# BelledonneCommunications/mediastreamer2

Measured on AMD Instinct MI355X. Metric: concurrent 48 kHz streams/node at <10 ms tick; Mpix/s YUV scale, higher is better.
Workload: dtype f32

## Files before the change

### mediastreamer2_amd/csrc/aec_steps.hpp

```cpp

template <int F_>
struct Wave {
	static constexpr int F = F_, K = F / 64, G = 64, NBL = 1;
	using Seq = WSeq<K>;
	__device__ static __forceinline__ int lane() { return threadIdx.x; }
	__device__ static __forceinline__ float first(float v) { return rdlane(v, 0); }
	__device__ static __forceinline__ float last(float v) { return rdlane(v, 63); }
	__device__ static __forceinline__ float shr1(float head, float v) {
		float t = __shfl_up(v, 1);
		if (threadIdx.x == 0) t = head;
		return t;
	}
	__device__ static __forceinline__ int any(bool p) { return __any(p); }
	template <typename Op>
	__device__ static __forceinline__ float tree(float v, Op op) { return wave_tree(v, op); }
	__device__ static __forceinline__ void dc_notch(const float (&in)[K], float radius, float den2, float &m0, float &m1, float (&out)[K]) {
		w_dc_notch<K>(in, radius, den2, m0, m1, out);
	}
	__device__ static __forceinline__ void deemphasis(const float (&d)[K], float &mem, float (&out)[K]) { w_deemphasis<K>(d, mem, out); }
	template <typename LL, typename LT>
	__device__ static __forceinline__ void rfft_forward(LL &L, const LT &T, float2 (&out)[K], const float *src = nullptr) {
		w_rfft_forward<F>(L, T, out, src);
	}
	template <typename LL, typename LT>
	__device__ static __forceinline__ void rfft_inverse(LL &L, const LT &T, const float2 (&in)[K]) { w_rfft_inverse<F>(L, T, in); }
	__device__ static __forceinline__ float band_total(const float (&vb)[NBL], float *) {
		float sum = 0;
#pragma unroll
		for (int i = 0; i < NB_BANDS; ++i) sum = sum + rdlane(vb[0], i);
		return sum;
	}
};

template <typename P, typename LL, typename LT>
__device__ __forceinline__ void far_end(LL &L, const LT &T, const float (&far)[P::K], const float (&xp)[P::K], float &memX, float (&xn)[P::K],
                                        float2 (&X0)[P::K], float &Sxx) {
	constexpr int K = P::K, F = P::F;
	const int e0 = P::lane() * K;
	float prev = P::shr1(memX, far[K - 1]);
#pragma unroll
	for (int k = 0; k < K; ++k) {
		xn[k] = far[k] - .9f * prev;
		prev = far[k];
	}
	memX = P::last(far[K - 1]);
	Sxx = P::Seq::inner_prod(xn, xn);
	WSYNC();
	store_vec<K>(L.tbuf + e0, xp);
	store_vec<K>(L.tbuf + F + e0, xn);
	P::rfft_forward(L, T, X0);
}

template <typename P>
__device__ __forceinline__ auto near_end(const float (&fin)[P::K], float radius, AecScalars &sc, float (&input)[P::K]) {
	constexpr int K = P::K;
	bool satl = false;
#pragma unroll
	for (int k = 0; k < K; ++k) satl |= (fin[k] <= -32000.f || fin[k] >= 32000.f);
	const auto any_sat = P::any(satl);
	const float den2 = (float)(radius * radius + .7 * (1 - radius) * (1 - radius));
	float v[K];
	P::dc_notch(fin, radius, den2, sc.notch0, sc.notch1, v);
	float vprev = P::shr1(sc.memD, v[K - 1]);
#pragma unroll
	for (int k = 0; k < K; ++k) {
		input[k] = v[k] - .9f * vprev;
		vprev = v[k];
	}
	sc.memD = P::last(v[K - 1]);
	return any_sat;
}

template <typename P>
__device__ __forceinline__ void bin_power(const float2 (&X)[P::K], float (&pw)[P::K], float &pw_F) {
	constexpr int K = P::K;
	const int e0 = P::lane() * K;
	float nyq = 0;
#pragma unroll
	for (int k = 0; k < K; ++k) {
		if (e0 + k == 0) {
			pw[k] = X[k].x * X[k].x;
			nyq = X[k].y * X[k].y;
		} else {
			pw[k] = X[k].x * X[k].x + X[k].y * X[k].y;
		}
	}
	pw_F = P::first(nyq);
}

template <typename P, typename TW, typename TX>
__device__ __forceinline__ void gradient(TW (&w)[P::K], const TX (&x)[P::K], float prop, const float2 (&E)[P::K], const float (&pp)[P::K], float pp_F) {
	constexpr int K = P::K;
	const int e0 = P::lane() * K;
#pragma unroll
	for (int k = 0; k < K; ++k) {
		const v2f xv = {x[k].x, x[k].y}, ev = {E[k].x, E[k].y};
		const float Wt = prop * pp[k];
		v2f st = pk_cmul_conj(xv, ev) * (v2f){Wt, Wt};
		if (k == 0) {
			const v2f dc = (xv * ev) * (v2f){Wt, prop * pp_F};
			if (e0 == 0) st = dc;
		}
		const v2f r = (v2f){w[k].x, w[k].y} + st;
		w[k].x = r.x, w[k].y = r.y;
	}
}

template <typename P, typename LL, typename LT, typename TW>
__device__ __forceinline__ void constrain(LL &L, const LT &T, TW (&wv)[P::K]) {
	constexpr int K = P::K, F = P::F;
	const int e0 = P::lane() * K;
	float2 w[K];
#pragma unroll
	for (int k = 0; k < K; ++k) w[k] = make_float2(wv[k].x, wv[k].y);
	P::rfft_inverse(L, T, w);
	float z[K];
#pragma unroll
	for (int k = 0; k < K; ++k) z[k] = 0.f;
	store_vec<K>(w_time(L) + F + e0, z);
	P::rfft_forward(L, T, w, w_time(L));
#pragma unroll
	for (int k = 0; k < K; ++k) wv[k].x = w[k].x, wv[k].y = w[k].y;
}

__device__ __forceinline__ bool two_path_update(AecScalars &sc, float Sff, float See, float Dbf) {
	sc.Davg1 = .6f * sc.Davg1 + .4f * (Sff - See);
	sc.Davg2 = .85f * sc.Davg2 + .15f * (Sff - See);
	sc.Dvar1 = .36f * sc.Dvar1 + (.4f * Sff) * (.4f * Dbf);
	sc.Dvar2 = .7225f * sc.Dvar2 + (.15f * Sff) * (.15f * Dbf);
	bool update_foreground = false;
	if ((Sff - See) * fabsf(Sff - See) > Sff * Dbf) update_foreground = true;
	else if (sc.Davg1 * fabsf(sc.Davg1) > .5f * sc.Dvar1) update_foreground = true;
	else if (sc.Davg2 * fabsf(sc.Davg2) > .25f * sc.Dvar2) update_foreground = true;
	if (update_foreground) {
		sc.fg_updates++;
		sc.Davg1 = sc.Davg2 = 0;
		sc.Dvar1 = sc.Dvar2 = 0;
	}
	return update_foreground;
}
template <typename P>
__device__ __forceinline__ void blend_foreground(const float *hann, float (&efg)[P::K], const float (&ybg)[P::K]) {
	constexpr int K = P::K, F = P::F;
	const int e0 = P::lane() * K;
	float h0[K], h1[K];
	load_vec<K>(hann + e0, h0);
	load_vec<K>(hann + F + e0, h1);
#pragma unroll
	for (int k = 0; k < K; ++k) efg[k] = h1[k] * efg[k] + h0[k] * ybg[k];
}
__device__ __forceinline__ bool two_path_reset(AecScalars &sc, float Sff, float See, float Dbf) {
	bool reset_background = false;
	if ((-(Sff - See)) * fabsf(Sff - See) > 4.f * (Sff * Dbf)) reset_background = true;
	if ((-sc.Davg1) * fabsf(sc.Davg1) > 4.f * sc.Dvar1) reset_background = true;
	if ((-sc.Davg2) * fabsf(sc.Davg2) > 4.f * sc.Dvar2) reset_background = true;
	if (reset_background) {
		sc.bg_resets++;
		sc.Davg1 = sc.Davg2 = 0;
		sc.Dvar1 = sc.Dvar2 = 0;
	}
	return reset_background;
}
template <typename P>
__device__ __forceinline__ void take_foreground(const float (&efg)[P::K], const float (&input)[P::K], float Sff, float (&ybg)[P::K], float (&e2)[P::K],
                                                float &See) {
#pragma unroll
	for (int k = 0; k < P::K; ++k) {
		ybg[k] = efg[k];
		e2[k] = input[k] - efg[k];
	}
	See = Sff;
}

template <typename P, typename TS>
__device__ __forceinline__ void output_and_correlations(AecScalars &sc, const float (&input)[P::K], const float (&efg)[P::K], const float (&e2)[P::K],
                                                        const float (&ybg)[P::K], TS any_sat, int (&out_i)[P::K], float &Sey, float &Syy, float &Sdd) {
	constexpr int K = P::K;
	{
		float d[K], tout[K];
#pragma unroll
		for (int k = 0; k < K; ++k) d[k] = input[k] - efg[k];
		P::deemphasis(d, sc.memE, tout);
#pragma unroll
// ... 359 lines not shown
```

### mediastreamer2_amd/csrc/aec_tick.hpp

```cpp

struct SmallLayout {
	int XPREV;
	int E;
	int POWER;
	int POWER1, EH, YH;
	int LASTY;
	int ECHON, INBUF, OUTBUF, NOISE, OLDPS, ZETA, S_, SMIN, STMP;
	int MISC;
	int PROP;
	int WNORM;
	int TAIL;
	int OLDPS_B;
	int ZETA_B;
	int FGNORM;
	int TOTAL;
};
__host__ __device__ constexpr SmallLayout small_layout(int F) {
	SmallLayout l{};
	l.XPREV = 0, l.E = F, l.POWER = 3 * F, l.POWER1 = 4 * F, l.EH = 5 * F, l.YH = 6 * F, l.LASTY = 7 * F;
	l.ECHON = 10 * F, l.INBUF = 11 * F, l.OUTBUF = 12 * F, l.NOISE = 13 * F, l.OLDPS = 14 * F, l.ZETA = 15 * F;
	l.S_ = 16 * F, l.SMIN = 17 * F, l.STMP = 18 * F, l.MISC = 19 * F;
	l.PROP = l.MISC, l.WNORM = l.MISC + 64, l.TAIL = l.MISC + 128, l.OLDPS_B = l.MISC + 136, l.ZETA_B = l.MISC + 160, l.FGNORM = l.MISC + 192;
	l.TOTAL = 19 * F + 256;
	return l;
// ... 162 lines not shown
enum { TICK_ROWS = 0, TICK_FIFO = 1, TICK_FIFO_RS = 2 };

template <int F, int MODE>
__global__ __launch_bounds__(64, F == 512 ? 1 : (F == 256 ? 2 : (F == 128 ? 3 : 4))) void aec_tick_kernel(AecArgs a) {
	__shared__ TLds<F> L;
	using SL = TickLayout<F>;
	using WP = Wave<F>;
	constexpr int N = 2 * F, K = F / 64;
	constexpr bool sched = MODE != TICK_ROWS;
	int s = a.first + blockIdx.x, par = 0;
	if (sched) {
		const unsigned c = blockIdx.x & 7u, i = blockIdx.x >> 3;
		par = a.ctl[TickOrder::GLOBAL + TickOrder::PARITY];
		const int front = a.ctl[c * TickOrder::STRIDE + TickOrder::PLACED + 2 * par], back = a.ctl[c * TickOrder::STRIDE + TickOrder::PLACED + 2 * par + 1];
		if (i >= (unsigned)front && i < (unsigned)(a.cap8 - back)) return;
		s = a.order[(size_t)par * 8 * a.cap8 + c * a.cap8 + i];
	}
	const int lane = threadIdx.x;
	const int e0 = lane * K;
	constexpr bool fifo = MODE != TICK_ROWS, folded = MODE == TICK_FIFO_RS;
	int nf, ref_frames = 0;
	int2 qm = make_int2(0, 0), qr = make_int2(0, 0), qo = make_int2(0, 0);
	bool mic_new = false, ref_new = false;
	if (fifo) {
		qm = a.fmic.pos[s], qr = a.fref.pos[s], qo = a.fout.pos[s];
		auto append = [&](const FifoView &q, int2 p, const int16_t *row, int len) -> bool {
			if (len <= 0) return false;
			if (p.y + len > q.cap) {
				if (lane == 0) atomicAdd(q.overflow, 1);
				return false;
			}
			int16_t *ring = q.ring + (size_t)s * q.cap;
			unsigned tail = (unsigned)p.x + (unsigned)p.y;
			if (tail >= (unsigned)q.cap) tail -= (unsigned)q.cap;
			if (((tail | (unsigned)len) & 7u) == 0 && (reinterpret_cast<uintptr_t>(row) & 15) == 0) {
				for (int i = lane; i < (len >> 3); i += 64) {
					unsigned w = tail + 8u * (unsigned)i;
					if (w >= (unsigned)q.cap) w -= (unsigned)q.cap;
					*reinterpret_cast<uint4 *>(ring + w) = *reinterpret_cast<const uint4 *>(row + 8 * i);
				}
			} else {
				for (int i = lane; i < len; i += 64) {
					unsigned w = tail + (unsigned)i;
					if (w >= (unsigned)q.cap) w -= (unsigned)q.cap;
					ring[w] = row[i];
				}
			}
			return true;
		};
		const int16_t *mic_row = folded ? nullptr : a.mic_tick + (size_t)s * a.mic_tick_stride;
		const int mlen = (a.run && !a.run[s]) ? 0 : a.tick_len;
		if (folded && mlen) {
			constexpr int RS_FILT = 48, RS_R = 8, RS_HIST = RS_FILT - 1;
			const int den = a.rs_den, in_len = a.rs_in_len;
			float *x = reinterpret_cast<float *>(L.zbuf);
			const int xn = ((RS_HIST + in_len + RS_R + 1) + 3) & ~3;
			int16_t *obuf = reinterpret_cast<int16_t *>(x + xn);
			float4 *tab4 = reinterpret_cast<float4 *>(obuf + ((in_len * den + 7) & ~7));
			const int hq = a.rs_hist_stride >> 2, nq = hq + (in_len >> 2);
			int16_t *hist = a.rs_hist + (size_t)s * a.rs_hist_stride;
			short4 v0 = make_short4(0, 0, 0, 0);
			if (lane < nq)
				v0 = *reinterpret_cast<const short4 *>(lane < hq ? hist + 4 * lane : a.rs_in + (size_t)s * a.rs_in_stride + 4 * (lane - hq));
			for (int i = lane; i < den * RS_FILT / 4; i += 64) tab4[i] = reinterpret_cast<const float4 *>(a.rs_table)[i];
			for (int i = RS_HIST + in_len + lane; i < xn; i += 64) x[i] = 0.f;
			if (lane < nq) {
				const int b = 4 * lane - (lane < hq ? 0 : 4 * hq - RS_HIST);
				if (lane < hq) {
					if (b + 0 < RS_HIST) x[b + 0] = (float)v0.x;
					if (b + 1 < RS_HIST) x[b + 1] = (float)v0.y;
					if (b + 2 < RS_HIST) x[b + 2] = (float)v0.z;
					if (b + 3 < RS_HIST) x[b + 3] = (float)v0.w;
				} else {
					x[b + 0] = (float)v0.x, x[b + 1] = (float)v0.y, x[b + 2] = (float)v0.z, x[b + 3] = (float)v0.w;
				}
			}
			wave_sync();
			const int nlanes = den * ((in_len + RS_R - 1) / RS_R);
			const bool on = lane < nlanes;
			const int tile = on ? lane / den : 0, ph = on ? lane - tile * den : 0, m0 = tile * RS_R;
			f2 acc2[RS_R / 2];
#pragma unroll
			for (int q = 0; q < RS_R / 2; ++q) acc2[q] = (f2){0.f, 0.f};
			fir_tile_rolled<RS_FILT, RS_R>(x + m0, reinterpret_cast<const float *>(tab4 + ph * (RS_FILT / 4)), acc2);
			if (on) {
#pragma unroll
				for (int r = 0; r < RS_R; ++r)
					if (m0 + r < in_len) obuf[(m0 + r) * den + ph] = rs_word2int((r & 1) ? acc2[r / 2].y : acc2[r / 2].x);
			}
			if (lane < hq) {
				const float *hx = x + in_len + 4 * lane;
				short4 h;
				h.x = (int16_t)hx[0], h.y = (int16_t)hx[1], h.z = (int16_t)hx[2], h.w = (int16_t)hx[3];
				*reinterpret_cast<short4 *>(hist + 4 * lane) = h;
			}
			wave_sync();
			mic_row = obuf;
		}
		int rlen = a.ref_len ? a.ref_len[s] : a.tick_len;
		rlen = rlen < 0 ? 0 : (rlen > a.tick_len ? a.tick_len : rlen);
		mic_new = append(a.fmic, qm, mic_row, mlen);
		ref_new = append(a.fref, qr, a.ref_tick + (size_t)s * a.ref_tick_stride, rlen);
		if (!ref_new) rlen = 0;
		nf = (qm.y + (mic_new ? a.tick_len : 0)) / F;
		if (nf > a.max_frames) nf = a.max_frames;
		ref_frames = (qr.y + rlen) / F;
		if (ref_frames > nf) ref_frames = nf;
		if (qo.y + nf * F > a.fout.cap) {
			if (lane == 0) atomicAdd(a.fout.overflow, 1);
			nf = 0;
		}
		if (sched && lane == 0) {
			const int keep = qm.y + (mic_new ? a.tick_len : 0) - nf * F;
			int next = (keep + a.tick_len) / F;
			if (next > a.max_frames) next = a.max_frames;
			const unsigned c = blockIdx.x & 7u, i = blockIdx.x >> 3, d = (c + i) & 7u;
			int *dst = a.order + (size_t)(par ^ 1) * 8 * a.cap8 + d * a.cap8;
			unsigned long long *placed = reinterpret_cast<unsigned long long *>(a.ctl + d * TickOrder::STRIDE + TickOrder::PLACED + 2 * (par ^ 1));
			const unsigned long long old = atomicAdd(placed, next >= 2 ? 1ull : (1ull << 32));
			const unsigned at = next >= 2 ? (unsigned)old : (unsigned)a.cap8 - 1u - (unsigned)(old >> 32);
			if (at < (unsigned)a.cap8) dst[at] = s;
		}
		if (lane == 0) {
			if (a.count_out) a.count_out[s] = (uint8_t)nf;
			const int rf = nf ? ref_frames : 0;
			a.fmic.pos[s] = make_int2((qm.x + nf * F) % a.fmic.cap, qm.y + (mic_new ? a.tick_len : 0) - nf * F);
			a.fref.pos[s] = make_int2((qr.x + rf * F) % a.fref.cap, qr.y + rlen - rf * F);
			a.fout.pos[s] = make_int2(qo.x, qo.y + nf * F);
		}
	} else {
		nf = a.count ? (int)a.count[s] : ((a.run && !a.run[s]) ? 0 : 1);
		if (nf > a.max_frames) nf = a.max_frames;
	}
	if (nf <= 0) return;
	auto ring_at = [&](const FifoView &q, int head, int p) -> int {
		unsigned at = (unsigned)head + (unsigned)p;
		if (at >= (unsigned)q.cap) at -= (unsigned)q.cap;
		if (at >= (unsigned)q.cap) at -= (unsigned)q.cap;
		return q.ring[(size_t)s * q.cap + at];
	};
	auto mic_at = [&](int f, int e) -> int {
		if (!fifo) return a.mic[(size_t)s * a.stride + f * F + e];
		const int p = f * F + e;
		if (folded || p < qm.y) return ring_at(a.fmic, qm.x, p);
		return a.mic_tick[(size_t)s * a.mic_tick_stride + (p - qm.y)];
	};
	auto ref_at = [&](int f, int e) -> int {
		if (!fifo) return a.ref[(size_t)s * a.stride + f * F + e];
		if (f >= ref_frames) return 0;
		const int p = f * F + e;
		if (p < qr.y) return ring_at(a.fref, qr.x, p);
		return a.ref_tick[(size_t)s * a.ref_tick_stride + (p - qr.y)];
	};
	auto out_ptr = [&](int f) -> int16_t * {
		if (!fifo) return a.out + (size_t)s * a.stride + f * F + e0;
		unsigned tail = (unsigned)(qo.x + qo.y) + (unsigned)(f * F);
		while (tail >= (unsigned)a.fout.cap) tail -= (unsigned)a.fout.cap;
		return a.fout.ring + (size_t)s * a.fout.cap + tail + e0;
	};
	const int M = a.M;
	float *sm = a.small + (size_t)s * a.small_stride;
	const rsrc_t rS = mk_rsrc(sm, (unsigned)a.small_stride * 4u);
	const rsrc_t rX = mk_rsrc(a.X + (size_t)s * (M + 1) * N, (unsigned)((M + 1) * N) * 4u);
	const rsrc_t rWF = mk_rsrc(a.WF + (size_t)s * 2 * M * N, (unsigned)(2 * M * N) * 4u);
	const unsigned HALF = (unsigned)(M * N) * 4u;
	const unsigned vb4 = (unsigned)e0 * 4u, vb8 = (unsigned)e0 * 8u;
	AecScalars sc = a.scal[s];
	unsigned wo = sc.wsel ? HALF : 0u, fo = HALF - wo;

#pragma unroll
	for (int k = 0; k < K; ++k) {
		L.tw[e0 + k] = a.t.tw[e0 + k];
		L.super[e0 + k] = a.t.super[e0 + k];
		L.perm[e0 + k] = a.t.perm[e0 + k];
	}
	if (lane < M) {
		L.prop[lane] = sm[SL::PROP + lane];
		L.wnorm[lane] = sm[SL::WNORM + lane];
	}
	float2 Eprev[K];
	float p1[K];
	bload_bins<K>(rS, vb8, SL::E * 4, Eprev);
	bload_vec<K>(rS, vb4, SL::POWER1 * 4, p1);
	{
		float t[K];
		bload_vec<K>(rS, vb4, SL::POWER * 4, t);
		store_vec<K>(L.pw + e0, t);
		bload_vec<K>(rS, vb4, SL::EH * 4, t);
		store_vec<K>(L.eh + e0, t);
		bload_vec<K>(rS, vb4, SL::YH * 4, t);
		store_vec<K>(L.yh + e0, t);
		bload_vec<K>(rS, vb4, (SL::LASTY + F) * 4, t);
		store_vec<K>(L.ly[0] + e0, t);
	}
	float pw_F = sm[SL::TAIL + 0], p1_F = sm[SL::TAIL + 1], eh_F = sm[SL::TAIL + 2], yh_F = sm[SL::TAIL + 3];
	bool prop_dirty = false;

	auto prep_far = [&](int f, const float (&xp)[K], float (&xn)[K], float2 (&X0)[K], float &Sxx) {
		float far[K];
#pragma unroll
		for (int k = 0; k < K; ++k) far[k] = (float)ref_at(f, e0 + k);
		far_end<WP>(L, a.t, far, xp, sc.memX, xn, X0, Sxx);
	};

	float2 X0[K], X0B[K];
	float Sxx = 0, SxxB = 0;
	{
		float xp[K], xa[K], xb[K];
		bload_vec<K>(rS, vb4, SL::XPREV * 4, xp);
		prep_far(0, xp, xa, X0, Sxx);
		if (nf > 1) {
			prep_far(1, xa, xb, X0B, SxxB);
			bstore_vec<K>(rS, vb4, SL::XPREV * 4, xb);
		} else {
			bstore_vec<K>(rS, vb4, SL::XPREV * 4, xa);
#pragma unroll
			for (int k = 0; k < K; ++k) X0B[k] = make_float2(0, 0);
		}
	}

	float2 spec2[K];
#pragma unroll
	for (int k = 0; k < K; ++k) spec2[k] = make_float2(0, 0);
	bool pendingFG = sc.fg_pending != 0, pendingBG = sc.bg_pending != 0;
	float fgnorm = lane < M ? sm[SL::FGNORM + lane] : 0.f;
	const bool postfilter = (a.flags & 1) != 0;
	float leakf[2] = {sc.leak_estimate, sc.leak_estimate};
	bool resetf[2] = {false, false};
	bool lazy1 = false;
	int jc1 = -1;
	float2 E1s[K];
	float p1s[K], p1s_F = 0.f;
#pragma unroll
	for (int k = 0; k < K; ++k) E1s[k] = make_float2(0, 0), p1s[k] = 0.f;

	for (int f = 0; f < nf; ++f) {
		const int head = (sc.xhead + M) % (M + 1);
		auto xoff = [&](int j) { return (unsigned)((head + j) % (M + 1)) * (unsigned)(F * 8); };
		v2f pre0[K], pre1[K], pre2[K], pre3[K];
		if (f == 0) {
#pragma unroll
			for (int k = 0; k < K; ++k) pre0[k] = pre1[k] = pre2[k] = pre3[k] = (v2f){0.f, 0.f};
		} else {
			bload_bins<K>(rX, vb8, xoff(1), pre0);
			bload_bins<K>(rX, vb8, xoff(2 < M ? 2 : M), pre1);
			const unsigned wpre = pendingBG ? fo : wo;
			bload_bins<K>(rWF, vb8, wpre, pre2);
			bload_bins<K>(rWF, vb8, wpre + (unsigned)(1 < M ? 1 : 0) * (unsigned)(F * 8), pre3);
		}
		int any_sat;
		{
			float input[K], fin[K];
#pragma unroll
			for (int k = 0; k < K; ++k) fin[k] = (float)mic_at(f, e0 + k);
			any_sat = near_end<WP>(fin, a.notch_radius, sc, input);
			store_vec<K>(L.input + e0, input);
		}
		sc.cancel_count++;
		sc.frames++;

		sc.xhead = head;
		bstore_bins<K>(rX, vb8, (unsigned)head * (F * 8), X0);
		float Xf[K], Xf_F;
		bin_power<WP>(X0, Xf, Xf_F);

		if (sc.adapted) {
			WSYNC();
			float p = sqrt_via_double(1.0f + (lane < M ? L.wnorm[lane] : 0.f));
			const float max_sum = wave_tree(lane < M ? p : 1.f, [](float x, float y) { return y > x ? y : x; });
			p = p + .1f * max_sum;
			float run = 1.f;
			for (int i = 0; i < M; ++i) run = dpp_shr1(1.f, run) + p;
			const float prop_sum = rdlane(run, M - 1);
			WSYNC();
			if (lane < M) L.prop[lane] = (.99f * p) / prop_sum;
			prop_dirty = true;
		}
		WSYNC();
		const bool do_grad = (sc.saturated == 0);
		if (!do_grad) sc.saturated--;

		const int jc = (M > 1) ? (sc.cancel_count % (M - 1)) + 1 : -1;
		float2 yfg[K], ybgs[K];
#pragma unroll
		for (int k = 0; k < K; ++k) yfg[k] = ybgs[k] = make_float2(0, 0);
		auto norm_of = [&](const auto (&w)[K], int j) {
			float nn = 0;
#pragma unroll
			for (int k = 0; k < K; ++k) nn += w[k].x * w[k].x + w[k].y * w[k].y;
			nn = wave_tree(nn, [](float x, float y) { return x + y; });
			if (lane == 0) L.wnorm[j] = nn;
		};
		if (f == 0) {
			const bool spec = nf > 1;
			v2f xj[K], xn[K], fg[K], wl[K], xm1[K];
#pragma unroll
			for (int k = 0; k < K; ++k) xj[k] = (v2f){X0[k].x, X0[k].y}, xm1[k] = (v2f){X0B[k].x, X0B[k].y};
			const bool carryFG = pendingFG, carryBG = pendingBG;
			pendingFG = pendingBG = false;
			const unsigned fsrc = carryFG ? wo : fo, wsrc = carryBG ? fo : wo, wdst = carryFG ? fo : wo;
			const bool lazy = spec && do_grad && !carryBG && !carryFG && M <= 32;
			bload_bins<K>(rX, vb8, xoff(1), xn);
			bload_bins<K>(rWF, vb8, fsrc, fg);
			bload_bins<K>(rWF, vb8, wsrc, wl);
			for (int j = 0; j < M; ++j) {
				v2f xn2[K], fg2[K], wl2[K];
				{
					const int jn = j + 1 < M ? j + 1 : j;
					bload_bins<K>(rX, vb8, xoff(jn + 1), xn2);
					bload_bins<K>(rWF, vb8, fsrc + (unsigned)jn * (F * 8), fg2);
					bload_bins<K>(rWF, vb8, wsrc + (unsigned)jn * (F * 8), wl2);
				}
				const bool aumdf = (j == 0 || j == jc);
				if (do_grad) gradient<WP>(wl, xn, L.prop[j], Eprev, p1, p1_F);
				if (aumdf) constrain<WP>(L, a.t, wl);
				if (lazy ? (aumdf || j == M - 1) : (do_grad || aumdf || carryBG || carryFG)) bstore_bins<K>(rWF, vb8, wdst + (unsigned)j * (F * 8), wl);
				cmac_bins<K>(yfg, xj, fg, e0);
				cmac_bins<K>(ybgs, xj, wl, e0);
				if (spec) cmac_bins<K>(spec2, xm1, fg, e0);
				norm_of(wl, j);
#pragma unroll
				for (int k = 0; k < K; ++k) xm1[k] = xj[k], xj[k] = xn[k], xn[k] = xn2[k], fg[k] = fg2[k], wl[k] = wl2[k];
			}
			if (carryFG) {
				const unsigned t = wo;
				wo = fo, fo = t;
				sc.wsel ^= 1;
			}
			if (lazy) {
				lazy1 = true;
				jc1 = jc;
				p1s_F = p1_F;
#pragma unroll
				for (int k = 0; k < K; ++k) E1s[k] = Eprev[k], p1s[k] = p1[k];
				WSYNC();
				if (lane < M) L.prop[32 + lane] = L.prop[lane];
				WSYNC();
			}
		} else {
			v2f xj[K], xn3[K];
			v2f(&xn)[K] = pre0, (&xn2)[K] = pre1, (&wl)[K] = pre2, (&wl2)[K] = pre3;
#pragma unroll
			for (int k = 0; k < K; ++k) xj[k] = (v2f){X0[k].x, X0[k].y};
			auto xclamp = [&](int i) { return xoff(i < M ? i : M); };
			auto wclamp = [&](int i) { return (unsigned)(i < M ? i : M - 1) * (unsigned)(F * 8); };
			const bool carryBG = pendingBG, carryFG = pendingFG;
			pendingBG = false;
			if (carryFG) {
#pragma unroll
				for (int k = 0; k < K; ++k) spec2[k] = make_float2(0, 0);
			}
			const unsigned wsrc = carryBG ? fo : wo, wdst = carryFG ? fo : wo;
			bload_bins<K>(rX, vb8, xclamp(3), xn3);
			__builtin_amdgcn_s_waitcnt(0x0F70);
			const bool redo = lazy1 && !carryBG;
			const bool keepW1 = redo && carryFG;
			auto block = [&](int j, v2f (&w)[K], const v2f (&xa)[K], const v2f (&xb)[K], const v2f (&xc)[K]) {
				if (redo && j != 0 && j != jc1 && j != M - 1) {
					gradient<WP>(w, xc, L.prop[32 + j], E1s, p1s, p1s_F);
					if (keepW1) bstore_bins<K>(rWF, vb8, wo + (unsigned)j * (F * 8), w);
				}
				if (carryFG) cmac_bins<K>(spec2, xa, w, e0);
				const bool aumdf = (j == 0 || j == jc);
				if (do_grad) gradient<WP>(w, xb, L.prop[j], Eprev, p1, p1_F);
				if (aumdf) constrain<WP>(L, a.t, w);
				if (do_grad || aumdf || carryBG || carryFG || lazy1) bstore_bins<K>(rWF, vb8, wdst + (unsigned)j * (F * 8), w);
				cmac_bins<K>(ybgs, xa, w, e0);
				norm_of(w, j);
			};
			if constexpr (F == 512) {
				for (int j = 0; j < M; ++j) {
					v2f xa[K], wa[K];
					bload_bins<K>(rX, vb8, xclamp(j + 4), xa);
					bload_bins<K>(rWF, vb8, wsrc + wclamp(j + 2), wa);
					block(j, wl, xj, xn, xn2);
#pragma unroll
					for (int k = 0; k < K; ++k) xj[k] = xn[k], xn[k] = xn2[k], xn2[k] = xn3[k], xn3[k] = xa[k], wl[k] = wl2[k], wl2[k] = wa[k];
				}
			} else {
			for (int j = 0; j < M; j += 2) {
				v2f xa[K], xb[K], wa[K], wb[K];
				bload_bins<K>(rX, vb8, xclamp(j + 4), xa);
				bload_bins<K>(rX, vb8, xclamp(j + 5), xb);
				bload_bins<K>(rWF, vb8, wsrc + wclamp(j + 2), wa);
				bload_bins<K>(rWF, vb8, wsrc + wclamp(j + 3), wb);
				block(j, wl, xj, xn, xn2);
				if (j + 1 < M) block(j + 1, wl2, xn, xn2, xn3);
#pragma unroll
				for (int k = 0; k < K; ++k) xj[k] = xn2[k], xn[k] = xn3[k], xn2[k] = xa[k], xn3[k] = xb[k], wl[k] = wa[k], wl2[k] = wb[k];
			}
			}
#pragma unroll
			for (int k = 0; k < K; ++k) yfg[k] = spec2[k];
			pendingFG = false;
			lazy1 = false;
			if (carryFG) {
				const unsigned t = wo;
				wo = fo, fo = t;
				sc.wsel ^= 1;
			}
		}

		float efg[K], ybg[K], e1[K], e2[K], dresp[K], input[K];
		w_rfft_inverse<F>(L, a.t, yfg);
		load_vec<K>(w_time(L) + F + e0, efg);
		load_vec<K>(L.input + e0, input);
#pragma unroll
		for (int k = 0; k < K; ++k) e1[k] = input[k] - efg[k];
		w_rfft_inverse<F>(L, a.t, ybgs);
		load_vec<K>(w_time(L) + F + e0, ybg);
#pragma unroll
		for (int k = 0; k < K; ++k) {
			e2[k] = input[k] - ybg[k];
			dresp[k] = efg[k] - ybg[k];
		}
		float Sff, Dbf, See;
		WSeq<K>::inner_prod3(e1, e1, dresp, dresp, e2, e2, Sff, Dbf, See);
		Dbf = 10 + Dbf;

		if (two_path_update(sc, Sff, See, Dbf)) {
			pendingFG = true;
			WSYNC();
			if (lane < M) fgnorm = L.wnorm[lane];
			blend_foreground<WP>(a.t.hann, efg, ybg);
		} else if (two_path_reset(sc, Sff, See, Dbf)) {
			pendingBG = true;
			WSYNC();
			if (lane < M) L.wnorm[lane] = fgnorm;
			take_foreground<WP>(efg, input, Sff, ybg, e2, See);
		}

		int out_i[K];
		float Sey, Syy, Sdd;
		output_and_correlations<WP>(sc, input, efg, e2, ybg, any_sat, out_i, Sey, Syy, Sdd);

		float2 Ecur[K], Ycur[K];
		error_spectra<WP>(L, a.t, e2, ybg, Ecur, Ycur);
		float Rf[K], Yf[K], Rf_F, Yf_F;
		bin_power<WP>(Ecur, Rf, Rf_F);
		bin_power<WP>(Ycur, Yf, Yf_F);
#pragma unroll
		for (int k = 0; k < K; ++k) Eprev[k] = Ecur[k];

		sanity_checks<WP>(sc, Sff, See, Sxx, Syy, Sdd, out_i);
		int16_t *op = out_ptr(f);
		auto emit = [&](const int (&o)[K]) {
#pragma unroll
			for (int k = 0; k < K; ++k) {
				if (postfilter) L.outf[f][e0 + k] = (int16_t)o[k];
				else op[k] = (int16_t)o[k];
			}
		};
		if (sc.screwed_up >= 50) {
			float z[K];
			float2 z2[K];
#pragma unroll
			for (int k = 0; k < K; ++k) z[k] = 0.f, z2[k] = make_float2(0, 0);
			for (int j = 0; j < M; ++j) {
				bstore_bins<K>(rWF, vb8, (unsigned)j * (F * 8), z2);
				bstore_bins<K>(rWF, vb8, HALF + (unsigned)j * (F * 8), z2);
			}
			for (int j = 0; j <= M; ++j) bstore_bins<K>(rX, vb8, (unsigned)j * (F * 8), z2);
#pragma unroll
			for (int k = 0; k < K; ++k) {
				p1[k] = 1.0f;
				Eprev[k] = make_float2(0, 0);
				spec2[k] = make_float2(0, 0);
			}
			lazy1 = false;
			store_vec<K>(L.pw + e0, z);
			store_vec<K>(L.eh + e0, z);
			store_vec<K>(L.yh + e0, z);
			store_vec<K>(L.ly[f + 1] + e0, z);
			pw_F = eh_F = yh_F = 0.f;
			p1_F = 1.0f;
			WSYNC();
			if (lane < M) L.wnorm[lane] = 0;
			fgnorm = 0.f;
			bstore_vec<K>(rS, vb4, SL::LASTY * 4, z);
			bstore_vec<K>(rS, vb4, (SL::LASTY + F) * 4, z);
			bstore_vec<K>(rS, vb4, (SL::LASTY + (2) * F) * 4, z);
			reset_scalars(sc);
			pendingFG = pendingBG = false;
			if (f) resetf[1] = true, leakf[1] = sc.leak_estimate;
			else resetf[0] = true, leakf[0] = sc.leak_estimate;
			emit(out_i);
			if (f + 1 < nf) {
				float xn[K];
				prep_far(f + 1, z, xn, X0, Sxx);
				bstore_vec<K>(rS, vb4, SL::XPREV * 4, xn);
			} else {
				bstore_vec<K>(rS, vb4, SL::XPREV * 4, z);
			}
			continue;
		}
		if (See < (float)(N * 100)) See = (float)(N * 100);
		float Sxx2 = Sxx + Sxx;

		float pw[K];
		load_vec<K>(L.pw + e0, pw);
		far_power<WP>(a, Xf, Xf_F, pw, pw_F);
		store_vec<K>(L.pw + e0, pw);
		float Ehd[K], Yhd[K], Ehd_F, Yhd_F;
		{
			float eh[K], yh[K];
			load_vec<K>(L.eh + e0, eh);
			load_vec<K>(L.yh + e0, yh);
			spectral_averages<WP>(a, Rf, Rf_F, Yf, Yf_F, eh, eh_F, yh, yh_F, Ehd, Ehd_F, Yhd, Yhd_F);
			store_vec<K>(L.eh + e0, eh);
			store_vec<K>(L.yh + e0, yh);
		}
		int m_here = M;
		asm volatile("" : "+s"(m_here));
		leak_and_steps<WP>(a, sc, m_here, Sxx2, See, Syy, Sey, Ehd, Ehd_F, Yhd, Yhd_F, Rf, Rf_F, Yf, Yf_F, pw, pw_F, p1, p1_F);

		{
			float ln[K], lprev[K];
			load_vec<K>(L.ly[f] + e0, lprev);
#pragma unroll
			for (int k = 0; k < K; ++k) ln[k] = sc.adapted ? (float)(mic_at(f, e0 + k) - out_i[k]) : lprev[k];
			store_vec<K>(L.ly[f + 1] + e0, ln);
		}
		if (f) leakf[1] = sc.leak_estimate;
		else leakf[0] = sc.leak_estimate;
		emit(out_i);
#pragma unroll
		for (int k = 0; k < K; ++k) X0[k] = X0B[k];
		Sxx = SxxB;
	}

	bstore_bins<K>(rS, vb8, SL::E * 4, Eprev);
	bstore_vec<K>(rS, vb4, SL::POWER1 * 4, p1);
	{
		float t[K];
		load_vec<K>(L.pw + e0, t);
		bstore_vec<K>(rS, vb4, SL::POWER * 4, t);
		load_vec<K>(L.eh + e0, t);
		bstore_vec<K>(rS, vb4, SL::EH * 4, t);
		load_vec<K>(L.yh + e0, t);
		bstore_vec<K>(rS, vb4, SL::YH * 4, t);
	}
	WSYNC();
	if (lane < M) {
		sm[SL::WNORM + lane] = L.wnorm[lane];
		sm[SL::FGNORM + lane] = fgnorm;
		if (prop_dirty) sm[SL::PROP + lane] = L.prop[lane];
	}
	{
		float lo[K], ln[K];
		load_vec<K>(L.ly[nf - 1] + e0, lo);
		load_vec<K>(L.ly[nf] + e0, ln);
		if (nf > 1 ? resetf[1] : resetf[0]) {
#pragma unroll
			for (int k = 0; k < K; ++k) lo[k] = 0.f;
		}
		bstore_vec<K>(rS, vb4, SL::LASTY * 4, lo);
		bstore_vec<K>(rS, vb4, (SL::LASTY + F) * 4, ln);
	}
	if (lane == 0) {
		sm[SL::TAIL + 0] = pw_F;
		sm[SL::TAIL + 1] = p1_F;
		sm[SL::TAIL + 2] = eh_F;
		sm[SL::TAIL + 3] = yh_F;
	}
	if (!postfilter) {
		sc.fg_pending = pendingFG ? 1 : 0, sc.bg_pending = pendingBG ? 1 : 0;
		if (lane == 0) a.scal[s] = sc;
		return;
	}
	WSYNC();

	PfState<WP> pf;
	pf_load<WP>(rS, vb4, a.t, pf);
	pf.old_ps_b[0] = pf.zeta_b[0] = 0;
	if (lane < NB_BANDS) {
		pf.old_ps_b[0] = sm[SL::OLDPS_B + lane];
		pf.zeta_b[0] = sm[SL::ZETA_B + lane];
	}
	for (int f = 0; f < nf; ++f) {
		{
			float lo[K], ln[K];
			load_vec<K>(L.ly[f] + e0, lo);
			load_vec<K>(L.ly[f + 1] + e0, ln);
			residual_echo<WP>(L, a.t, pf, lo, ln, f ? resetf[1] : resetf[0], f ? leakf[1] : leakf[0]);
		}
		float xcur[K];
#pragma unroll
		for (int k = 0; k < K; ++k) xcur[k] = (float)L.outf[f][e0 + k];
		int out_f[K];
		postfilter_frame<WP>(L, a.t, a.t, L.vec(), L.band(), sc, pf, xcur, out_f);
		int16_t *op = out_ptr(f);
#pragma unroll
		for (int k = 0; k < K; ++k) op[k] = (int16_t)out_f[k];
		WSYNC();
	}
	pf_store<WP>(rS, vb4, pf);
	if (lane < NB_BANDS) {
		sm[SL::OLDPS_B + lane] = pf.old_ps_b[0];
		sm[SL::ZETA_B + lane] = pf.zeta_b[0];
	}

	sc.fg_pending = pendingFG ? 1 : 0, sc.bg_pending = pendingBG ? 1 : 0;
	if (lane == 0) a.scal[s] = sc;
}
```

### mediastreamer2_amd/csrc/aec_wave.hpp

```cpp

template <int F>
struct alignas(16) WLds {
	float2 zbuf[F];
	float tbuf[2 * F];
	float spec[2 * F];
	float2 tw[F], super[F];
	uint16_t perm[F];
	float prop[64];
	float band[4 * NB_BANDS + 8];
	float vec[F];
};

#define WSYNC() __syncthreads()

template <typename LT>
__device__ __forceinline__ float *w_time(LT &L) { return reinterpret_cast<float *>(L.zbuf); }

template <int F, typename LT>
__device__ void w_cfft(LT &L, const AecTables &T, const float2 *src, bool inverse) {
	constexpr int K = F / 64;
	const int lane = threadIdx.x;
	float2 val[K];
#pragma unroll
	for (int k = 0; k < K; ++k) {
// ... 109 lines not shown
				const float2 s3 = make_float2(s0.x + s2.x, s0.y + s2.y);
				const float2 s4 = make_float2(s0.x - s2.x, s0.y - s2.y);
				Fo[2 * m] = make_float2(f0.x - s3.x, f0.y - s3.y);
				f0.x += s3.x;
				f0.y += s3.y;
				Fo[0] = f0;
				if (inverse) {
					Fo[m] = make_float2(s5.x - s4.y, s5.y + s4.x);
					Fo[3 * m] = make_float2(s5.x + s4.y, s5.y - s4.x);
				} else {
					Fo[m] = make_float2(s5.x + s4.y, s5.y - s4.x);
					Fo[3 * m] = make_float2(s5.x - s4.y, s5.y + s4.x);
				}
			}
		};
		if constexpr (F > 256) {
#pragma unroll 1
			for (int bf = lane; bf < F / p; bf += 64) butterfly(bf);
		} else {
			if (lane < F / p) butterfly(lane);
		}
		WSYNC();
	}
}

template <int K>
__device__ __forceinline__ void load_bins(const float2 *p, float2 (&v)[K]);
template <int K>
__device__ __forceinline__ void store_bins(float2 *p, const float2 (&v)[K]);

template <int F, typename LT>
__device__ __forceinline__ void w_rfft_forward_bins(LT &L, float2 (&out)[F / 64]) {
	constexpr int K = F / 64;
	const int lane = threadIdx.x;
	const float scale = 1.f / (2 * F);
#pragma unroll
	for (int k = 0; k < K; ++k) {
		const int b = lane * K + k;
		if (b == 0) {
			const float2 t0 = L.zbuf[0];
			out[k] = make_float2((t0.x + t0.y) * scale, (t0.x - t0.y) * scale);
		} else {
			const bool upper = b >= F - b;
			const int kk = upper ? F - b : b;
			const float2 a = L.zbuf[kk], c = L.zbuf[F - kk];
			const float2 sw = L.super[kk];
			const v2f av = {a.x, a.y}, cv = {c.x, c.y};
			v2f f1, f2;
			asm("v_pk_add_f32 %0, %1, %2 neg_hi:[0,1]" : "=v"(f1) : "v"(av), "v"(cv));
			asm("v_pk_add_f32 %0, %1, %2 neg_lo:[0,1]" : "=v"(f2) : "v"(av), "v"(cv));
			v2f tw = pk_cmul(f2, (v2f){sw.x, sw.y});
			const unsigned flip = upper ? 0x80000000u : 0u;
			f1.y = __uint_as_float(__float_as_uint(f1.y) ^ flip);
			tw.x = __uint_as_float(__float_as_uint(tw.x) ^ flip);
			const v2f r = (((v2f){.5f, .5f}) * (f1 + tw)) * (v2f){scale, scale};
			out[k] = make_float2(r.x, r.y);
		}
	}
}
template <int F, typename LT>
__device__ __attribute__((noinline)) void w_rfft_forward_lds(LT &L, const AecTables &T, const float *src) {
	constexpr int K = F / 64;
	w_cfft<F>(L, T, reinterpret_cast<const float2 *>(src), false);
	float2 r[K];
	w_rfft_forward_bins<F>(L, r);
	WSYNC();
	store_bins<K>(L.zbuf + threadIdx.x * K, r);
}

template <int F, typename LT>
__device__ void w_rfft_forward(LT &L, const AecTables &T, float2 (&out)[F / 64], const float *src = nullptr) {
	if (src == nullptr) src = L.tbuf;
	constexpr int K = F / 64;
	WSYNC();
	if constexpr (F == 512) {
		w_rfft_forward_lds<F>(L, T, src);
		load_bins<K>(L.zbuf + threadIdx.x * K, out);
	} else {
		w_cfft<F>(L, T, reinterpret_cast<const float2 *>(src), false);
		w_rfft_forward_bins<F>(L, out);
	}
	WSYNC();
}

template <int F, typename LT>
__device__ __forceinline__ void w_rfft_inverse_tail(LT &L, const AecTables &T) {
	constexpr int K = F / 64;
	const int lane = threadIdx.x;
	float2 *tmp = reinterpret_cast<float2 *>(L.tbuf);
	float2 t[K];
#pragma unroll
	for (int k = 0; k < K; ++k) {
		const int i = lane * K + k;
		if (i == 0) {
			t[k] = make_float2(L.spec[0] + L.spec[1], L.spec[0] - L.spec[1]);
		} else {
			const bool upper = i >= F - i;
			const int kk = upper ? F - i : i;
			const v2f fk = {L.spec[2 * kk], L.spec[2 * kk + 1]};
			const v2f s2 = {L.spec[2 * (F - kk)], L.spec[2 * (F - kk) + 1]};
			const float2 sw = L.super[kk];
			const v2f sv = {sw.x, sw.y};
			v2f fek, d, p, q, fok;
			asm("v_pk_add_f32 %0, %1, %2 neg_hi:[0,1]" : "=v"(fek) : "v"(fk), "v"(s2));
			asm("v_pk_add_f32 %0, %1, %2 neg_lo:[0,1]" : "=v"(d) : "v"(fk), "v"(s2));
			asm("v_pk_mul_f32 %0, %1, %2 op_sel_hi:[1,0]" : "=v"(p) : "v"(d), "v"(sv));
			asm("v_pk_mul_f32 %0, %1, %2 op_sel:[1,1] op_sel_hi:[0,1] neg_lo:[0,1] neg_hi:[0,1]" : "=v"(q) : "v"(d), "v"(sv));
			asm("v_pk_add_f32 %0, %1, %2 neg_lo:[0,1]" : "=v"(fok) : "v"(p), "v"(q));
			const unsigned flip = upper ? 0x80000000u : 0u;
			fok.x = __uint_as_float(__float_as_uint(fok.x) ^ flip);
			fok.y = __uint_as_float(__float_as_uint(fok.y) ^ flip);
			v2f r = fek + fok;
			r.y = __uint_as_float(__float_as_uint(r.y) ^ flip);
			t[k] = make_float2(r.x, r.y);
		}
	}
	WSYNC();
#pragma unroll
	for (int k = 0; k < K; ++k) tmp[lane * K + k] = t[k];
	WSYNC();
	w_cfft<F>(L, T, tmp, true);
}
template <int F, typename LT>
__device__ __attribute__((noinline)) void w_rfft_inverse_lds(LT &L, const AecTables &T) {
	w_rfft_inverse_tail<F>(L, T);
}

template <int F, typename LT>
__device__ void w_rfft_inverse(LT &L, const AecTables &T, const float2 (&in)[F / 64]) {
	constexpr int K = F / 64;
	const int lane = threadIdx.x;
	WSYNC();
#pragma unroll
	for (int k = 0; k < K; ++k) {
		L.spec[2 * (lane * K + k)] = in[k].x;
		L.spec[2 * (lane * K + k) + 1] = in[k].y;
	}
	WSYNC();
	if constexpr (F == 512) w_rfft_inverse_lds<F>(L, T);
	else w_rfft_inverse_tail<F>(L, T);
}


__device__ __forceinline__ float dpp_shr1_zero(float v) {
	return __int_as_float(__builtin_amdgcn_update_dpp(0, __float_as_int(v), 0x138, 0xf, 0xf, true));
}
__device__ __forceinline__ float dpp_shr1(float first, float v) {
	return __int_as_float(__builtin_amdgcn_update_dpp(__float_as_int(first), __float_as_int(v), 0x138, 0xf, 0xf, false));
}
__device__ __forceinline__ float dpp_shl1(float last, float v) {
	return __int_as_float(__builtin_amdgcn_update_dpp(__float_as_int(last), __float_as_int(v), 0x130, 0xf, 0xf, false));
}

template <typename Op>
__device__ __forceinline__ float wave_tree(float v, Op op) {
	auto dpp = [](float x, auto ctrl) {
		return __int_as_float(__builtin_amdgcn_update_dpp(__float_as_int(x), __float_as_int(x), decltype(ctrl)::value, 0xf, 0xf, false));
	};
	v = op(v, dpp(v, std::integral_constant<int, 0xB1>{}));
	v = op(v, dpp(v, std::integral_constant<int, 0x4E>{}));
	v = op(v, dpp(v, std::integral_constant<int, 0x141>{}));
	v = op(v, dpp(v, std::integral_constant<int, 0x140>{}));
	const float r0 = rdlane(v, 0), r1 = rdlane(v, 16), r2 = rdlane(v, 32), r3 = rdlane(v, 48);
	return op(op(r0, r1), op(r2, r3));
}

template <int K>
struct WSeq {
	static constexpr int KP = K >= 2 ? K / 2 : 1;
	__device__ static void pairs(const float (&x)[K], const float (&y)[K], float (&part)[KP]) {
		if constexpr (K == 1) {
			const float pr = x[0] * y[0];
			const float nb = __int_as_float(__builtin_amdgcn_update_dpp(0, __float_as_int(pr), 0xB1, 0xf, 0xf, true));
			float p = 0;
			p = p + pr;
			p = p + nb;
			part[0] = (threadIdx.x & 1) ? -0.0f : p;
		} else {
#pragma unroll
			for (int k = 0; k < K; k += 2) {
				float p = 0;
				p = p + x[k] * y[k];
				p = p + x[k + 1] * y[k + 1];
				part[k / 2] = p;
			}
		}
	}
	template <int NC>
	__device__ static void chain_up(const float (&part)[NC][KP], float (&sum)[NC]) {
		float s[NC];
#pragma unroll
		for (int c = 0; c < NC; ++c) s[c] = 0;
#pragma unroll 4
		for (int l = 0; l < 64; ++l) {
#pragma unroll
			for (int c = 0; c < NC; ++c) {
				s[c] = dpp_shr1_zero(s[c]) + part[c][0];
#pragma unroll
				for (int k = 1; k < KP; ++k) s[c] = s[c] + part[c][k];
			}
		}
#pragma unroll
		for (int c = 0; c < NC; ++c) sum[c] = rdlane(s[c], 63);
	}
	__device__ static float inner_prod(const float (&x)[K], const float (&y)[K]) {
		float part[1][KP], sum[1];
		pairs(x, y, part[0]);
		chain_up<1>(part, sum);
		return sum[0];
	}
	__device__ static void inner_prod3(const float (&x0)[K], const float (&y0)[K], const float (&x1)[K], const float (&y1)[K],
	                                   const float (&x2)[K], const float (&y2)[K], float &r0, float &r1, float &r2) {
		float part[3][KP], sum[3];
		pairs(x0, y0, part[0]);
		pairs(x1, y1, part[1]);
		pairs(x2, y2, part[2]);
		chain_up<3>(part, sum);
		r0 = sum[0], r1 = sum[1], r2 = sum[2];
	}
	__device__ static void dot_desc2(float init0, const float (&a0)[K], const float (&b0)[K], float init1, const float (&a1)[K],
	                                 const float (&b1)[K], float &r0, float &r1) {
		float p0[K], p1[K];
#pragma unroll
		for (int k = 0; k < K; ++k) p0[k] = a0[k] * b0[k], p1[k] = a1[k] * b1[k];
		float s0 = init0, s1 = init1;
#pragma unroll 4
		for (int l = 0; l < 64; ++l) {
			v2f t = {dpp_shl1(init0, s0), dpp_shl1(init1, s1)};
#pragma unroll
			for (int k = K - 1; k >= 0; --k) t = t + (v2f){p0[k], p1[k]};
			s0 = t.x, s1 = t.y;
		}
		r0 = rdlane(s0, 0), r1 = rdlane(s1, 0);
	}
};

template <bool HI>
__device__ __forceinline__ void notch_sample(v2f rc, v2f pair, float vin, float &a0, float &a1, float &out) {
	v2f vo, tu, am;
	vo.x = a0 + vin;
	asm("v_pk_mul_f32 %0, %1, %2 op_sel_hi:[1,0]" : "=v"(tu) : "v"(rc), "v"(vo));
	if constexpr (HI) asm("v_pk_add_f32 %0, %1, %2 op_sel:[0,1] op_sel_hi:[1,1] neg_lo:[0,1] neg_hi:[1,0]" : "=v"(am) : "v"(tu), "v"(pair));
	else asm("v_pk_add_f32 %0, %1, %2 op_sel_hi:[1,0] neg_lo:[0,1] neg_hi:[1,0]" : "=v"(am) : "v"(tu), "v"(pair));
	a0 = __builtin_fmaf(2.f, am.x, a1);
	a1 = am.y;
	out = tu.x;
}
template <int K>
__device__ __forceinline__ void w_dc_notch(const float (&in)[K], float radius, float den2, float &m0io, float &m1io, float (&out)[K]) {
	const float i0 = m0io, i1 = m1io;
	float m0 = i0, m1 = i1;
	const v2f rc = {radius, den2};
	constexpr int NP = (K + 1) / 2;
	v2f pr[NP];
#pragma unroll
	for (int k = 0; k < K; ++k) {
		if (k & 1) pr[k / 2].y = in[k];
		else pr[k / 2].x = in[k];
	}
#pragma unroll 2
	for (int l = 0; l < 64; ++l) {
		float a0 = dpp_shr1(i0, m0), a1 = dpp_shr1(i1, m1);
#pragma unroll
		for (int k = 0; k < K; ++k) {
			if (k & 1) notch_sample<true>(rc, pr[k / 2], in[k], a0, a1, out[k]);
			else notch_sample<false>(rc, pr[k / 2], in[k], a0, a1, out[k]);
		}
		m0 = a0, m1 = a1;
	}
	m0io = rdlane(m0, 63);
	m1io = rdlane(m1, 63);
}

template <int K>
__device__ __forceinline__ void w_deemphasis(const float (&d)[K], float &memio, float (&out)[K]) {
	const float init = memio;
	float m = init;
#pragma unroll 2
	for (int l = 0; l < 64; ++l) {
		float a = dpp_shr1(init, m);
#pragma unroll
		for (int k = 0; k < K; ++k) {
			const float t = d[k] + .9f * a;
			a = t;
			out[k] = t;
		}
		m = a;
	}
	memio = rdlane(m, 63);
}

template <int K>
__device__ __forceinline__ void load_vec(const float *p, float (&v)[K]) {
	if constexpr (K == 4) {
		const float4 t = *reinterpret_cast<const float4 *>(p);
		v[0] = t.x, v[1] = t.y, v[2] = t.z, v[3] = t.w;
	} else if constexpr (K == 2) {
		const float2 t = *reinterpret_cast<const float2 *>(p);
		v[0] = t.x, v[1] = t.y;
	} else if constexpr (K == 8) {
		const float4 t = *reinterpret_cast<const float4 *>(p), u = *reinterpret_cast<const float4 *>(p + 4);
		v[0] = t.x, v[1] = t.y, v[2] = t.z, v[3] = t.w, v[4] = u.x, v[5] = u.y, v[6] = u.z, v[7] = u.w;
	} else {
		v[0] = *p;
	}
}
template <int K>
__device__ __forceinline__ void store_vec(float *p, const float (&v)[K]) {
	if constexpr (K == 4) *reinterpret_cast<float4 *>(p) = make_float4(v[0], v[1], v[2], v[3]);
	else if constexpr (K == 2) *reinterpret_cast<float2 *>(p) = make_float2(v[0], v[1]);
	else if constexpr (K == 8) {
		*reinterpret_cast<float4 *>(p) = make_float4(v[0], v[1], v[2], v[3]);
		*reinterpret_cast<float4 *>(p + 4) = make_float4(v[4], v[5], v[6], v[7]);
	} else *p = v[0];
}
template <int K>
__device__ __forceinline__ void load_bins(const float2 *p, float2 (&v)[K]) {
	if constexpr (K == 1) {
		v[0] = *p;
	} else {
#pragma unroll
		for (int k = 0; k < K; k += 2) {
			const float4 t = *reinterpret_cast<const float4 *>(p + k);
			v[k] = make_float2(t.x, t.y);
			v[k + 1] = make_float2(t.z, t.w);
		}
	}
}
template <int K>
__device__ __forceinline__ void store_bins(float2 *p, const float2 (&v)[K]) {
	if constexpr (K == 1) {
		*p = v[0];
	} else {
#pragma unroll
		for (int k = 0; k < K; k += 2) *reinterpret_cast<float4 *>(p + k) = make_float4(v[k].x, v[k].y, v[k + 1].x, v[k + 1].y);
	}
}
```

Baseline: 114,700.

## Restrict wave-serial recurrence chains to one 16-lane row at a time

Replaces the 64-step wave-wide serial scans (prefix chain, descending dot, DC notch, deemphasis) with a row_chain helper. It loops over four 16-lane rows, runs 16 DPP row-shift steps only in the active row, then carries the head value across rows with readlane. The point is to cut the number of steps each lane executes, since the old scan stepped the whole wave 64 times. It also rolls the paired filter-block loop into a non-unrolled inner loop to reduce code size and register pressure. It adds a WaveTail policy with an opaque lane index for the postfilter. The divergent row branches and extra readlanes could add overhead.

```diff
diff --git a/mediastreamer2_amd/csrc/aec_steps.hpp b/mediastreamer2_amd/csrc/aec_steps.hpp
--- a/mediastreamer2_amd/csrc/aec_steps.hpp
+++ b/mediastreamer2_amd/csrc/aec_steps.hpp
@@ -29,6 +29,15 @@
 #pragma unroll
 		for (int i = 0; i < NB_BANDS; ++i) sum = sum + rdlane(vb[0], i);
 		return sum;
+	}
+};
+
+template <int F_>
+struct WaveTail : Wave<F_> {
+	__device__ static __forceinline__ int lane() {
+		int l = threadIdx.x;
+		asm("" : "+v"(l));
+		return l;
 	}
 };
 
diff --git a/mediastreamer2_amd/csrc/aec_tick.hpp b/mediastreamer2_amd/csrc/aec_tick.hpp
--- a/mediastreamer2_amd/csrc/aec_tick.hpp
+++ b/mediastreamer2_amd/csrc/aec_tick.hpp
@@ -338,7 +338,7 @@
 		if (p < qr.y) return ring_at(a.fref, qr.x, p);
 		return a.ref_tick[(size_t)s * a.ref_tick_stride + (p - qr.y)];
 	};
-	auto out_ptr = [&](int f) -> int16_t * {
+	auto out_ptr = [&](int f, int e0) -> int16_t * {
 		if (!fifo) return a.out + (size_t)s * a.stride + f * F + e0;
 		unsigned tail = (unsigned)(qo.x + qo.y) + (unsigned)(f * F);
 		while (tail >= (unsigned)a.fout.cap) tail -= (unsigned)a.fout.cap;
@@ -570,10 +570,15 @@
 				bload_bins<K>(rX, vb8, xclamp(j + 5), xb);
 				bload_bins<K>(rWF, vb8, wsrc + wclamp(j + 2), wa);
 				bload_bins<K>(rWF, vb8, wsrc + wclamp(j + 3), wb);
-				block(j, wl, xj, xn, xn2);
-				if (j + 1 < M) block(j + 1, wl2, xn, xn2, xn3);
-#pragma unroll
-				for (int k = 0; k < K; ++k) xj[k] = xn2[k], xn[k] = xn3[k], xn2[k] = xa[k], xn3[k] = xb[k], wl[k] = wa[k], wl2[k] = wb[k];
+				const int jend = j + 2 < M ? j + 2 : M;
+#pragma unroll 1
+				for (int i = j; i < jend; ++i) {
+					block(i, wl, xj, xn, xn2);
+#pragma unroll
+					for (int k = 0; k < K; ++k) xj[k] = xn[k], xn[k] = xn2[k], xn2[k] = xn3[k], wl[k] = wl2[k];
+				}
+#pragma unroll
+				for (int k = 0; k < K; ++k) xn2[k] = xa[k], xn3[k] = xb[k], wl[k] = wa[k], wl2[k] = wb[k];
 			}
 			}
 #pragma unroll
@@ -629,7 +634,7 @@
 		for (int k = 0; k < K; ++k) Eprev[k] = Ecur[k];
 
 		sanity_checks<WP>(sc, Sff, See, Sxx, Syy, Sdd, out_i);
-		int16_t *op = out_ptr(f);
+		int16_t *op = out_ptr(f, e0);
 		auto emit = [&](const int (&o)[K]) {
 #pragma unroll
 			for (int k = 0; k < K; ++k) {
@@ -756,8 +761,9 @@
 	}
 	WSYNC();
 
-	PfState<WP> pf;
-	pf_load<WP>(rS, vb4, a.t, pf);
+	using WT = WaveTail<F>;
+	PfState<WT> pf;
+	pf_load<WT>(rS, vb4, a.t, pf);
 	pf.old_ps_b[0] = pf.zeta_b[0] = 0;
 	if (lane < NB_BANDS) {
 		pf.old_ps_b[0] = sm[SL::OLDPS_B + lane];
@@ -768,19 +774,19 @@
 			float lo[K], ln[K];
 			load_vec<K>(L.ly[f] + e0, lo);
 			load_vec<K>(L.ly[f + 1] + e0, ln);
-			residual_echo<WP>(L, a.t, pf, lo, ln, f ? resetf[1] : resetf[0], f ? leakf[1] : leakf[0]);
+			residual_echo<WT>(L, a.t, pf, lo, ln, f ? resetf[1] : resetf[0], f ? leakf[1] : leakf[0]);
 		}
 		float xcur[K];
 #pragma unroll
 		for (int k = 0; k < K; ++k) xcur[k] = (float)L.outf[f][e0 + k];
 		int out_f[K];
-		postfilter_frame<WP>(L, a.t, a.t, L.vec(), L.band(), sc, pf, xcur, out_f);
-		int16_t *op = out_ptr(f);
+		postfilter_frame<WT>(L, a.t, a.t, L.vec(), L.band(), sc, pf, xcur, out_f);
+		int16_t *op = out_ptr(f, WT::lane() * K);
 #pragma unroll
 		for (int k = 0; k < K; ++k) op[k] = (int16_t)out_f[k];
 		WSYNC();
 	}
-	pf_store<WP>(rS, vb4, pf);
+	pf_store<WT>(rS, vb4, pf);
 	if (lane < NB_BANDS) {
 		sm[SL::OLDPS_B + lane] = pf.old_ps_b[0];
 		sm[SL::ZETA_B + lane] = pf.zeta_b[0];
diff --git a/mediastreamer2_amd/csrc/aec_wave.hpp b/mediastreamer2_amd/csrc/aec_wave.hpp
--- a/mediastreamer2_amd/csrc/aec_wave.hpp
+++ b/mediastreamer2_amd/csrc/aec_wave.hpp
@@ -285,6 +285,33 @@
 	return __int_as_float(__builtin_amdgcn_update_dpp(__float_as_int(last), __float_as_int(v), 0x130, 0xf, 0xf, false));
 }
 
+template <int NS, bool DESC, int UNROLL, typename Step>
+__device__ __forceinline__ void row_chain(float (&s)[NS], Step step) {
+	float head[NS];
+#pragma unroll
+	for (int c = 0; c < NS; ++c) head[c] = s[c];
+#pragma unroll 1
+	for (int r = 0; r < 4; ++r) {
+		const int row = DESC ? 3 - r : r;
+		if ((int)(threadIdx.x >> 4) == row) {
+#pragma unroll UNROLL
+			for (int l = 0; l < 16; ++l) {
+				float a[NS];
+#pragma unroll
+				for (int c = 0; c < NS; ++c)
+					a[c] = __int_as_float(__builtin_amdgcn_update_dpp(__float_as_int(head[c]), __float_as_int(s[c]), DESC ? 0x101 : 0x111, 0xf, 0xf, false));
+				step(a);
+#pragma unroll
+				for (int c = 0; c < NS; ++c) s[c] = a[c];
+			}
+		}
+#pragma unroll
+		for (int c = 0; c < NS; ++c) head[c] = rdlane(s[c], DESC ? 16 * row : 16 * row + 15);
+	}
+#pragma unroll
+	for (int c = 0; c < NS; ++c) s[c] = head[c];
+}
+
 template <typename Op>
 __device__ __forceinline__ float wave_tree(float v, Op op) {
 	auto dpp = [](float x, auto ctrl) {
@@ -321,20 +348,15 @@
 	}
 	template <int NC>
 	__device__ static void chain_up(const float (&part)[NC][KP], float (&sum)[NC]) {
-		float s[NC];
-#pragma unroll
-		for (int c = 0; c < NC; ++c) s[c] = 0;
-#pragma unroll 4
-		for (int l = 0; l < 64; ++l) {
+#pragma unroll
+		for (int c = 0; c < NC; ++c) sum[c] = 0;
+		row_chain<NC, false, 4>(sum, [&](float (&a)[NC]) {
 #pragma unroll
 			for (int c = 0; c < NC; ++c) {
-				s[c] = dpp_shr1_zero(s[c]) + part[c][0];
-#pragma unroll
-				for (int k = 1; k < KP; ++k) s[c] = s[c] + part[c][k];
-			}
-		}
-#pragma unroll
-		for (int c = 0; c < NC; ++c) sum[c] = rdlane(s[c], 63);
+#pragma unroll
+				for (int k = 0; k < KP; ++k) a[c] = a[c] + part[c][k];
+			}
+		});
 	}
 	__device__ static float inner_prod(const float (&x)[K], const float (&y)[K]) {
 		float part[1][KP], sum[1];
@@ -356,15 +378,14 @@
 		float p0[K], p1[K];
 #pragma unroll
 		for (int k = 0; k < K; ++k) p0[k] = a0[k] * b0[k], p1[k] = a1[k] * b1[k];
-		float s0 = init0, s1 = init1;
-#pragma unroll 4
-		for (int l = 0; l < 64; ++l) {
-			v2f t = {dpp_shl1(init0, s0), dpp_shl1(init1, s1)};
+		float s[2] = {init0, init1};
+		row_chain<2, true, 4>(s, [&](float (&a)[2]) {
+			v2f t = {a[0], a[1]};
 #pragma unroll
 			for (int k = K - 1; k >= 0; --k) t = t + (v2f){p0[k], p1[k]};
-			s0 = t.x, s1 = t.y;
-		}
-		r0 = rdlane(s0, 0), r1 = rdlane(s1, 0);
+			a[0] = t.x, a[1] = t.y;
+		});
+		r0 = s[0], r1 = s[1];
 	}
 };
 
@@ -381,8 +402,6 @@
 }
 template <int K>
 __device__ __forceinline__ void w_dc_notch(const float (&in)[K], float radius, float den2, float &m0io, float &m1io, float (&out)[K]) {
-	const float i0 = m0io, i1 = m1io;
-	float m0 = i0, m1 = i1;
 	const v2f rc = {radius, den2};
 	constexpr int NP = (K + 1) / 2;
 	v2f pr[NP];
@@ -391,36 +410,29 @@
 		if (k & 1) pr[k / 2].y = in[k];
 		else pr[k / 2].x = in[k];
 	}
-#pragma unroll 2
-	for (int l = 0; l < 64; ++l) {
-		float a0 = dpp_shr1(i0, m0), a1 = dpp_shr1(i1, m1);
+	float m[2] = {m0io, m1io};
+	row_chain<2, false, 2>(m, [&](float (&a)[2]) {
 #pragma unroll
 		for (int k = 0; k < K; ++k) {
-			if (k & 1) notch_sample<true>(rc, pr[k / 2], in[k], a0, a1, out[k]);
-			else notch_sample<false>(rc, pr[k / 2], in[k], a0, a1, out[k]);
-		}
-		m0 = a0, m1 = a1;
-	}
-	m0io = rdlane(m0, 63);
-	m1io = rdlane(m1, 63);
+			if (k & 1) notch_sample<true>(rc, pr[k / 2], in[k], a[0], a[1], out[k]);
+			else notch_sample<false>(rc, pr[k / 2], in[k], a[0], a[1], out[k]);
+		}
+	});
+	m0io = m[0], m1io = m[1];
 }
 
 template <int K>
 __device__ __forceinline__ void w_deemphasis(const float (&d)[K], float &memio, float (&out)[K]) {
-	const float init = memio;
-	float m = init;
-#pragma unroll 2
-	for (int l = 0; l < 64; ++l) {
-		float a = dpp_shr1(init, m);
+	float m[1] = {memio};
+	row_chain<1, false, 2>(m, [&](float (&a)[1]) {
 #pragma unroll
 		for (int k = 0; k < K; ++k) {
-			const float t = d[k] + .9f * a;
-			a = t;
+			const float t = d[k] + .9f * a[0];
+			a[0] = t;
 			out[k] = t;
 		}
-		m = a;
-	}
-	memio = rdlane(m, 63);
+	});
+	memio = m[0];
 }
 
 template <int K>
```

New measurement: 114,700. No clear change (+0.0%).
